# junghoseong/aircombat-selfplay

Measured on AMD Instinct MI355X. Metric: agent-steps/sec, higher is better.
Workload: dtype f32

## Files before the change

__graft_entry__.py:

```python
import os
import subprocess
import sys

ROOT = os.path.dirname(os.path.abspath(__file__))
PKG = os.path.join(ROOT, "aircombat-selfplay_amd")
HIPCC = os.environ.get("HIPCC", "/opt/rocm/bin/hipcc")


def _stale(out, srcs):
    if not os.path.exists(out):
        return True
    t = os.path.getmtime(out)
    return any(os.path.getmtime(s) > t for s in srcs if os.path.exists(s))


HIP_FLAGS = ["--offload-arch=gfx950", "-O3", "-std=c++17",
             "-fno-hip-fp32-correctly-rounded-divide-sqrt", "-fgpu-flush-denormals-to-zero",
             "-fno-slp-vectorize"]


def build_hip(force=False):
    csrc = os.path.join(PKG, "csrc")
    src = os.path.join(csrc, "aircombat.hip")
    gen = os.path.join(ROOT, "tools", "gen_split_tick.py")
    if subprocess.run([sys.executable, gen, "--check"]).returncode != 0:
        subprocess.check_call([sys.executable, gen], stdout=subprocess.DEVNULL)
    deps = [os.path.join(csrc, f) for f in sorted(os.listdir(csrc))] + [
        os.path.join(ROOT, "include", "aircombat.h"), os.path.join(ROOT, "include", "aircombat_buffer.h"), os.path.join(ROOT, "include", "aircombat_epoch.h"), os.path.join(ROOT, "include", "aircombat_rollout.h"),
        os.path.join(ROOT, "include", "aircombat_rollout_share.h"), os.path.join(ROOT, "include", "aircombat_eval.h"), os.path.join(ROOT, "include", "aircombat_league.h"), os.path.join(ROOT, "include", "aircombat_record.h"), os.path.join(ROOT, "include", "aircombat_spawn.h"), os.path.join(ROOT, "include", "aircombat_mutual.h"),
        os.path.join(ROOT, "tools", "check_exec_restore.py"), os.path.join(ROOT, "tools", "check_hidden_loads.py"),
        os.path.join(ROOT, "tools", "check_shuffle_discipline.py"), gen, os.path.abspath(__file__)]
    out = os.path.join(PKG, "libaircombat_hip.so")
    if force or _stale(out, deps):
        srcs = [os.path.join(csrc, f) for f in sorted(os.listdir(csrc)) if f.endswith((".hip", ".hpp"))]
        lint = subprocess.run([sys.executable, os.path.join(ROOT, "tools", "check_shuffle_discipline.py")] + srcs, capture_output=True, text=True)
        if lint.returncode != 0:
            raise RuntimeError("shuffle on the right of a short-circuit operator in the HIP sources:\n" + lint.stdout)
        bdir = os.path.join(PKG, "build")
        os.makedirs(bdir, exist_ok=True)
        asm = os.path.join(bdir, "aircombat_gfx950.s")
        subprocess.check_call([HIPCC] + HIP_FLAGS + ["--cuda-device-only", "-S", "-o", asm, src], stderr=subprocess.DEVNULL)
        lint = subprocess.run([sys.executable, os.path.join(ROOT, "tools", "check_exec_restore.py"), asm], capture_output=True, text=True)
        if lint.returncode != 0:
            raise RuntimeError("gfx950 code-generation hazard in the HIP extension, refusing to build it:\n" + lint.stdout)
        lint = subprocess.run([sys.executable, os.path.join(ROOT, "tools", "check_hidden_loads.py"), asm], capture_output=True, text=True)
        if lint.returncode != 0:
            raise RuntimeError("a hand-placed action-row load has its registers touched before its wait, refusing to build:\n" + lint.stdout)
        tmp = out + ".tmp"
        subprocess.check_call([HIPCC] + HIP_FLAGS + ["-fPIC", "-shared", "-o", tmp, src, "-lhsa-runtime64"])
        os.replace(tmp, out)
    return out


def build_oracle(force=False):
    out = os.path.join(ROOT, "oracle", "_build", "liboracle.so")
    srcs = [os.path.join(ROOT, "oracle", f) for f in
            ("f16_fdm.c", "geodesy.c", "combat_env.c", "state_bridge.c", "bench_port.c", "lowlevel_actor.c", "f16_fdm.h", "geodesy.h", "combat_env.h", "f16_tables.h")]
    if force or _stale(out, srcs):
        subprocess.check_call(["make", "-C", os.path.join(ROOT, "oracle")] + (["-B"] if force else []), stdout=subprocess.DEVNULL)
    return out


def build():
    build_hip()
    build_oracle()
    if ROOT not in sys.path:
        sys.path.insert(0, ROOT)
    import aircombat_selfplay_amd as pkg
    pkg.load_library()


def smoke():
    if ROOT not in sys.path:
        sys.path.insert(0, ROOT)
    import numpy as np
    import aircombat_selfplay_amd as pkg
    from oracle import oracle as O

    build_oracle()
    cfg = pkg.default_config("singlecombat")
    env = pkg.HipVecEnv(cfg, 8, device_id=0)
    ref = O.OracleVecEnv(O.config_from_ac(cfg), 8)
    obs = env.reset()
    robs = ref.reset()
    assert np.allclose(obs, robs, rtol=1e-4, atol=2e-4), np.abs(obs - robs).max()
    rng = np.random.default_rng(0)
    for _ in range(5):
        act = np.stack([rng.integers(0, n, size=(8, 2)) for n in (41, 41, 41, 30)], axis=-1).astype(np.float32)
        obs, rew, done, info = env.step(act)
        robs, rrew, rdone, _ = ref.step(act)
        assert np.allclose(obs, robs, rtol=1e-3, atol=1e-3), np.abs(obs - robs).max()
        assert np.allclose(rew, rrew, rtol=1e-3, atol=2e-3), np.abs(rew - rrew).max()
        assert (done == rdone).all()
    env.close()
    print("smoke ok: HIP step matches the oracle on 8 envs x 5 steps")


if __name__ == "__main__":
    build()
    if len(sys.argv) > 1 and sys.argv[1] == "smoke":
        smoke()
```

aircombat-selfplay_amd/capi.py:

```python
import ctypes as C
import os

AC_MAX_AGENTS = 8
AC_MAX_MISSILES_PER_AGENT = 4
AC_STATE_LEN = 128

AC_TASK_HEADING, AC_TASK_SINGLECOMBAT, AC_TASK_DODGE_MISSILE, AC_TASK_SHOOT_MISSILE, AC_TASK_MULTICOMBAT = 0, 1, 2, 3, 4
AC_TASK_SCENARIO1, AC_TASK_SCENARIO_NVN, AC_TASK_WVR, AC_TASK_MANEUVER = 5, 6, 7, 8
AC_ALIVE, AC_CRASH, AC_SHOTDOWN = 0, 1, 2
AC_CTL_FAST, AC_CTL_FP32 = 0, 1
AC_CENT_EXPLICIT, AC_CENT_ENV_SHARE = 0, 1
AC_POOL_PPO, AC_POOL_MAPPO = 0, 1


class HipExtensionMissing(RuntimeError):
    pass


(AC_BUF_OBS, AC_BUF_SHARE_OBS, AC_BUF_ACTIONS, AC_BUF_REWARDS, AC_BUF_MASKS, AC_BUF_BAD_MASKS, AC_BUF_ACTIVE_MASKS, AC_BUF_LOGP,
 AC_BUF_VALUES, AC_BUF_RETURNS, AC_BUF_RNN_ACTOR, AC_BUF_RNN_CRITIC, AC_BUF_ADVANTAGES, AC_BUF_NFIELDS) = range(14)
AC_EPOCH_FIELDS = ("obs", "share_obs", "actions", "masks", "active_masks", "action_log_probs", "advantages", "returns", "value_preds",
                   "rnn_states_actor", "rnn_states_critic")
AC_EPOCH_NFIELDS = len(AC_EPOCH_FIELDS)

# ... 156 lines not shown
               [(n, C.c_void_p) for n in ("rewards", "info", "stage", "spawned", "episode", "ret_acc", "wins", "played", "return_sum", "index")]


AC_MI_HIDDEN, AC_MI_WIDTH, AC_MI_MAX_ACT, AC_MI_MAX_OBS = 128, 256, 12, 128
AC_MI_WEIGHTS = ("p_w0", "p_b0", "p_w1", "p_b1", "p_w2", "p_b2", "q_w0", "q_b0", "q_w1", "q_b1", "q_w2", "q_b2")


class AcMiScore(C.Structure):
    _fields_ = [(n, C.c_int32) for n in ("E", "na", "T", "obs_dim", "act_dim", "hidden", "s0", "n", "add")] + [("ratio", C.c_float)] + \
               [(n, C.c_void_p) for n in ("OBS", "ACTIONS", "RNN_ACTOR", "REWARDS") + AC_MI_WEIGHTS + ("r_int", "mse")]


class AcMiGather(C.Structure):
    _fields_ = [(n, C.c_int32) for n in ("E", "na", "T", "obs_dim", "act_dim", "hidden", "m", "pad_")] + \
               [(n, C.c_void_p) for n in ("OBS", "ACTIONS", "RNN_ACTOR", "times", "X", "Y")]


AC_LATE_FRACTION_DEFAULT, AC_LATE_BUDGET_DEFAULT = 1.0, 400000


class AcLateStats(C.Structure):
    _fields_ = [("steps", C.c_int64), ("retries", C.c_int64), ("last_retries", C.c_int32), ("last_late", C.c_int32), ("retry_steps", C.c_int64), ("lowered", C.c_int64), ("disabled", C.c_int64), ("fraction", C.c_double), ("timed_steps", C.c_int64),
                ("copy_before_us", C.c_double), ("dispatch_us", C.c_double), ("copy_after_us", C.c_double), ("wait_us", C.c_double)]


AC_PPO_STAT_LOSS, AC_PPO_STAT_POLICY_LOSS, AC_PPO_STAT_VALUE_LOSS, AC_PPO_STAT_ENTROPY_LOSS, AC_PPO_STAT_RATIO_MEAN, AC_PPO_STAT_DENOMINATOR = range(6)
AC_PPO_NSTAT = 8

AC_PROBE_IN, AC_PROBE_OUT, AC_PROBE_MAX_ROWS = 6, 12, 1 << 22
AC_PROBE_OPS = ("fx_rcp", "fx_rsqrt", "fx_sqrt", "fx_sqrt_both", "fx_sincos", "atan2_fast", "acos_fast", "pow_pos", "tanh_fast", "atanh_fast",
                "sigmoid_f", "tanh_f", "atmosphere", "pitot", "vcas", "in_range_deg", "in_range_rad", "slew", "tef_kinematic", "seek",
                "posture_fn", "missile_height_f", "missile_height_d", "neu_height64", "locate", "locate_fast")
AC_PROBE_MSL_IN, AC_PROBE_MSL_TGT, AC_PROBE_MSL_OUT = 16, 7, 16
AC_PROBE_MSL_MAX_ROWS, AC_PROBE_MSL_MAX_TICKS, AC_PROBE_MSL_MAX_CELLS = 512, 4200, 1 << 19

_p = C.c_void_p
SIGNATURES = {
    "ac_state_field_name": (C.c_char_p, [C.c_int]),
    "ac_create": (C.c_int, [C.POINTER(AcConfig), C.c_int32, C.c_int32, C.c_uint64, C.POINTER(_p)]),
    "ac_destroy": (C.c_int, [_p]),
    "ac_obs_dim": (C.c_int, [_p]),
    "ac_act_dim": (C.c_int, [_p]),
    "ac_num_envs": (C.c_int, [_p]),
    "ac_num_agents": (C.c_int, [_p]),
    "ac_reset": (C.c_int, [_p, _p]),
    "ac_step": (C.c_int, [_p, _p, _p, _p, _p, _p]),
    "ac_host_buffers": (C.c_int, [_p, C.c_int32, C.POINTER(_p), C.POINTER(_p), C.POINTER(_p), C.POINTER(_p), C.POINTER(_p)]),
    "ac_host_set_detach": (C.c_int, [_p, C.c_int32]),
    "ac_host_set_free": (None, [_p, _p, _p, _p, _p]),
    "ac_step_host_async": (C.c_int, [_p, C.c_int32]),
    "ac_step_host_wait": (C.c_int, [_p]),
    "ac_step_host": (C.c_int, [_p, C.c_int32]),
    "ac_step_host_actions": (C.c_int, [_p, C.c_int32, _p, C.c_size_t]),
    "ac_late_config": (C.c_int, [_p, C.c_double, C.c_int32, C.c_int32, C.c_int32]),
    "ac_late_stats": (C.c_int, [_p, _p]),
    "ac_order_after": (C.c_int, [_p, _p]),
    "ac_order_before": (C.c_int, [_p, _p]),
    "ac_step_async_device": (C.c_int, [_p, _p]),
    "ac_device_buffers": (C.c_int, [_p, C.POINTER(_p), C.POINTER(_p), C.POINTER(_p), C.POINTER(_p), C.POINTER(_p)]),
    "ac_stream": (_p, [_p]),
    "ac_dispatch_path": (C.c_char_p, [_p]),
    "ac_sync": (C.c_int, [_p]),
    "ac_get_state": (C.c_int, [_p, C.c_int32, C.c_int32, C.POINTER(C.c_double)]),
    "ac_set_state": (C.c_int, [_p, C.c_int32, C.c_int32, C.POINTER(C.c_double)]),
    "ac_set_status": (C.c_int, [_p, C.c_int32, C.c_int32, C.c_int32]),
    "ac_get_entity": (C.c_int, [_p, C.c_int32, C.c_int32, C.POINTER(C.c_double)]),
    "ac_get_missile": (C.c_int, [_p, C.c_int32, C.c_int32, C.c_int32, C.POINTER(C.c_double)]),
    "ac_get_missile_target": (C.c_int, [_p, C.c_int32, C.c_int32, C.c_int32, C.POINTER(C.c_int32)]),
    "ac_timing_begin": (C.c_int, [_p]),
    "ac_timing_end": (C.c_int, [_p, C.POINTER(C.c_float)]),
    "ac_step_timed_device": (C.c_int, [_p, _p, C.POINTER(C.c_float), C.POINTER(C.c_float)]),
    "ac_state_checksum": (C.c_int, [_p, C.POINTER(C.c_uint64)]),
    "ac_munitions_in_flight": (C.c_int, [_p, C.POINTER(C.c_int32)]),
    "ac_seed_envs": (C.c_int, [_p, _p]),
    "ac_get_heading_state": (C.c_int, [_p, C.c_int32, _p]),
    "ac_pin_host_buffer": (C.c_int, [_p, _p, C.c_int64]),
    "ac_unpin_host_buffer": (C.c_int, [_p, _p]),
    "ac_load_controller": (C.c_int, [_p, _p, C.c_int64]),
    "ac_split_f16x2": (C.c_int, [_p, C.c_int64, _p, _p]),
    "ac_split_bf16x3": (C.c_int, [_p, C.c_int64, _p, _p, _p]),
    "ac_controller_precision": (C.c_int, [_p]),
    "ac_controller_forward": (C.c_int, [C.c_int32, C.c_int32, _p, C.c_int64, C.c_int64, _p, _p, _p, _p]),
    "ac_selftest_missile_walk": (C.c_int, [C.c_int32, _p]),
    "ac_probe_math": (C.c_int, [_p, C.c_int32, C.c_int64, _p, _p]),
    "ac_probe_missile": (C.c_int, [_p, C.c_int32, C.c_int32, C.c_int32, C.c_int32, _p, _p, _p]),
    "ac_get_controller_state": (C.c_int, [_p, C.c_int32, C.c_int32, _p, _p]),
    "ac_set_controller_state": (C.c_int, [_p, C.c_int32, C.c_int32, _p]),
    "ac_snapshot_bytes": (C.c_int, [_p, C.POINTER(C.c_int64)]),
    "ac_snapshot_header": (C.c_int, [_p, _p]),
    "ac_snapshot_save": (C.c_int, [_p, _p]),
    "ac_snapshot_load": (C.c_int, [_p, _p]),
    "ac_snapshot_save_host": (C.c_int, [_p, _p, C.c_int64]),
    "ac_snapshot_load_host": (C.c_int, [_p, _p, C.c_int64]),
    "ac_clone_envs": (C.c_int, [_p, _p, _p, C.c_int32]),
    "ac_snapshot_load_envs": (C.c_int, [_p, _p, _p, C.c_int32]),
    "ac_get_obs": (C.c_int, [_p, _p]),
    "ac_snapshot_checksum": (C.c_int, [_p, C.POINTER(C.c_uint64)]),
    "ac_policy_blob_floats": (C.c_int, [_p, C.POINTER(C.c_int64), C.POINTER(C.c_int64)]),
    "ac_policy_create": (C.c_int, [C.c_int32, _p, C.POINTER(_p)]),
    "ac_policy_destroy": (C.c_int, [_p]),
    "ac_policy_load": (C.c_int, [_p, _p, C.c_int64, _p, C.c_int64]),
    "ac_policy_load_device": (C.c_int, [_p, _p, _p, C.c_int64, _p, C.c_int64]),
    "ac_policy_load_refused": (C.c_int, [_p, _p, C.POINTER(C.c_int32), C.POINTER(C.c_int32)]),
    "ac_policy_packed": (C.c_int, [_p, C.c_int32, C.POINTER(_p), C.POINTER(C.c_int64)]),
    "ac_policy_get_actions": (C.c_int, [_p, _p, _p, _p, _p, _p, _p, C.c_int32, C.c_uint64, C.c_uint64, _p, _p, _p, _p, _p]),
    "ac_policy_draw_host": (C.c_int, [C.c_uint64, C.c_uint64, C.c_int64, C.c_int64, C.c_int32, _p]),
# ... 170 lines not shown
```

aircombat-selfplay_amd/csrc/aircombat.hip:

```cpp
#include <hip/hip_runtime.h>
#include <stdint.h>
#include <stdio.h>
#include <string.h>
#include <string>
#include <vector>
#include <cmath>
#include <algorithm>
#include <chrono>
#include "../../include/aircombat.h"
#include "../../include/aircombat_buffer.h"
#include "clk_stamps.hpp"
#include "f16_device.hpp"
#include "f16_split.hpp"

using f16::State;
using f16::Derived;
using f16::Tab;
using f16::clampf;

#define AC_F_FIELDS(X)                                                                                           \
  X(vx) X(vy) X(vz) X(q0) X(q1) X(q2) X(q3) X(wp) X(wq) X(wr) X(hv1x) X(hv1y) X(hv1z) X(hv2x) X(hv2y) X(hv2z)   \
  X(ha1x) X(ha1y) X(ha1z) X(wdx) X(wdy) X(wdz) X(aix) X(aiy) X(aiz) X(bax) X(bay) X(baz) X(da) X(de) X(dr)       \
  X(thr) X(pin_r) X(pin_p) X(pin_y) X(pi_r) X(pi_p) X(pi_y) X(tef) X(ail) X(elev) X(sbdeg) X(alpha) X(mach)      \
  X(qc) X(vg) X(ap) X(aq) X(ar) X(npx) X(npy) X(npz) X(n1) X(n2) X(n2norm) X(ff) X(tank0) X(tank1)
// ... 2063 lines not shown
    const size_t Npad = ((size_t)h->N + 63) / 64 * 64;
    const size_t act_bytes = (sizeof(float) * Npad * h->act_dim + 63) / 64 * 64;
    HIP_OK(hipHostMalloc((void**)&hs.act, act_bytes + sizeof(int) * late::HDR_WORDS, hipHostMallocDefault));
    hs.hdr = reinterpret_cast<int*>(reinterpret_cast<char*>(hs.act) + act_bytes);
    memset(hs.hdr, 0, sizeof(int) * late::HDR_WORDS);
    hs.tag = 0; hs.plain_rows = false;
    HIP_OK(hipHostMalloc((void**)&hs.obs, sizeof(float) * Npad * h->obs_dim, hipHostMallocDefault));
    HIP_OK(hipHostMalloc((void**)&hs.rew, sizeof(float) * Npad, hipHostMallocDefault));
    HIP_OK(hipHostMalloc((void**)&hs.done, Npad, hipHostMallocDefault));
    HIP_OK(hipHostMalloc((void**)&hs.info, sizeof(int) * (Npad / h->A), hipHostMallocDefault));
    memset(hs.act, 0, sizeof(float) * Npad * h->act_dim); memset(hs.obs, 0, sizeof(float) * Npad * h->obs_dim);
    memset(hs.rew, 0, sizeof(float) * Npad); memset(hs.done, 0, Npad); memset(hs.info, 0, sizeof(int) * (Npad / h->A));
    h->have_hs[set] = true;
  }
  if (actions) *actions = hs.act;
  if (obs) *obs = hs.obs;
  if (rewards) *rewards = hs.rew;
  if (dones) *dones = hs.done;
  if (info) *info = hs.info;
  return 0;
}
int ac_host_set_detach(ac_env_t* h, int32_t set) {
  if (!h || set < 0 || set >= AC_HOST_SETS || !h->have_hs[set]) return fail("ac_host_set_detach: no such set");
  if (host_entry(h)) return -1;
  HIP_OK(hipSetDevice(h->device));
  HIP_OK(hipStreamSynchronize(h->stream));
  h->have_hs[set] = false;
  memset(&h->hs[set], 0, sizeof h->hs[set]);
  return 0;
}
void ac_host_set_free(void* actions, void* obs, void* rewards, void* dones, void* info) {
  (void)hipHostFree(actions); (void)hipHostFree(obs); (void)hipHostFree(rewards); (void)hipHostFree(dones); (void)hipHostFree(info);
}
int ac_step_host_async(ac_env_t* h, int32_t set) {
  if (!h || set < 0 || set >= AC_HOST_SETS) return fail("ac_step_host_async: bad argument");
  if (!h->have_hs[set]) return fail("ac_step_host_async: call ac_host_buffers for this set first");
  HIP_OK(hipSetDevice(h->device));
  return host_step(h, set);
}
int ac_step_host_wait(ac_env_t* h) {
  if (!h) return fail("ac_step_host_wait: null handle");
  if (h->aql.in_flight) {
    if (aql_settle(h)) return -1;
  } else {
    HIP_OK(hipStreamSynchronize(h->stream));
    h->stream_dirty = false;
  }
  return check_nonfinite(h, "ac_step_host_wait");
}
int ac_step_host(ac_env_t* h, int32_t set) {
  if (ac_step_host_async(h, set)) return -1;
  return ac_step_host_wait(h);
}
int ac_step_host_actions(ac_env_t* h, int32_t set, const float* actions, size_t n_floats) {
  if (!h || !actions || set < 0 || set >= AC_HOST_SETS) return fail("ac_step_host_actions: bad argument");
  if (!h->have_hs[set]) return fail("ac_step_host_actions: call ac_host_buffers for this set first");
  if (n_floats != (size_t)h->N * h->act_dim) return fail("ac_step_host_actions: n_floats is not num_envs * num_agents * act_dim");
  HIP_OK(hipSetDevice(h->device));
  h->late_set = -1;
  if (host_step(h, set, actions)) return -1;
  const int ls = h->late_set;
  std::chrono::steady_clock::time_point t0;
  if (ls >= 0 && h->late_timing) t0 = std::chrono::steady_clock::now();
  const int rc = ac_step_host_wait(h);
  if (ls >= 0) {
    ac_late_stats_t& st = h->late_stats;
    if (h->late_timing) st.wait_us += std::chrono::duration<double, std::micro>(std::chrono::steady_clock::now() - t0).count();
    st.last_retries = *(volatile int*)&h->hs[ls].hdr[late::HDR_RETRIES];
    st.retries += st.last_retries;
    st.retry_steps += st.last_retries != 0;
    st.steps += 1;
    h->late_win_steps += 1;
    h->late_win_retry += st.last_retries != 0;
    if (h->late_win_steps == AC_LATE_WINDOW) {
      if (h->late_win_retry > AC_LATE_WINDOW_MAX_RETRY_STEPS) {
        h->late_fraction -= 0.25;
        st.lowered += 1;
        if (h->late_fraction <= 0.0) { h->late_fraction = 0.0; h->late_off = true; st.disabled = 1; }
      }
      h->late_win_steps = h->late_win_retry = 0;
    }
    st.fraction = h->late_fraction;
    h->late_set = -1;
  }
  return rc;
}
int ac_late_config(ac_env_t* h, double fraction, int32_t budget, int32_t delay_us, int32_t timing) {
  if (!h) return fail("ac_late_config: null handle");
  if (fraction > 1.0 || budget > (1 << 24)) return fail("ac_late_config: fraction above 1 or budget above 2^24 tries");
  if (host_entry(h)) return -1;
  if (fraction >= 0.0) { h->late_fraction = fraction; h->late_off = false; h->late_stats.disabled = 0; h->late_win_steps = h->late_win_retry = 0; }
  if (budget >= 0) h->late_budget = budget;
  if (delay_us >= 0) h->late_delay_us = delay_us;
  if (timing >= 0) h->late_timing = timing != 0;
  return 0;
}
int ac_late_stats(ac_env_t* h, ac_late_stats_t* out) {
  if (!h || !out) return fail("ac_late_stats: null argument");
  *out = h->late_stats;
  out->fraction = h->late_fraction;
  return 0;
}

int ac_order_after(ac_env_t* h, void* producer_stream) {
  if (!h) return fail("ac_order_after: null handle");
  if (host_entry(h)) return -1;
  HIP_OK(hipSetDevice(h->device));
  HIP_OK(hipEventRecord(h->ev_order, (hipStream_t)producer_stream));
  HIP_OK(hipStreamWaitEvent(h->stream, h->ev_order, 0));
  return 0;
}
int ac_order_before(ac_env_t* h, void* consumer_stream) {
  if (!h) return fail("ac_order_before: null handle");
  if (host_entry(h)) return -1;
  HIP_OK(hipSetDevice(h->device));
  HIP_OK(hipEventRecord(h->ev_order, h->stream));
  HIP_OK(hipStreamWaitEvent((hipStream_t)consumer_stream, h->ev_order, 0));
  return 0;
}

int ac_step_async_device(ac_env_t* h, const float* d_actions) {
  if (!h) return fail("ac_step_async_device: null handle");
  if (host_entry(h)) return -1;
  HIP_OK(hipSetDevice(h->device));
  return launch_step(h, d_actions);
}
int ac_device_buffers(ac_env_t* h, float** d_actions, float** d_obs, float** d_rewards, uint8_t** d_dones, int32_t** d_info) {
  if (!h) return fail("ac_device_buffers: null handle");
  if (d_actions) *d_actions = h->d_actions;
  if (d_obs) *d_obs = h->dp.obs;
  if (d_rewards) *d_rewards = h->dp.rew;
  if (d_dones) *d_dones = h->dp.done;
  if (d_info) *d_info = h->dp.info;
  return 0;
}
void* ac_stream(ac_env_t* h) {
  if (!h) return nullptr;
  (void)host_entry(h);
// ... 496 lines not shown
```

aircombat-selfplay_amd/vec_env.py:

```python
import ctypes as C
import os
import sys

import numpy as np

from .capi import (AcConfig, AC_STATE_LEN, AC_TASK_HEADING, AC_TASK_SINGLECOMBAT, AC_TASK_SHOOT_MISSILE, AC_TASK_MULTICOMBAT, AC_TASK_SCENARIO1,
                   AC_TASK_SCENARIO_NVN, AC_CTL_FAST, AC_CTL_FP32, load_library)
from . import capi
from .config import config_from_yaml, default_config
from .snapshot import EnvSnapshot, MultiSnapshot, SnapshotMismatch, check_compatible, decode_header

DONE_MESSAGES = {
    0: "", 1: "altitude is too low", 2: "is on an extreme state", 3: "acceleration is too high", 4: "has been shot down",
    5: "has crashed", 6: "mission completed", 7: "step limits", 8: "unreached heading",
}


class _Box:

    def __init__(self, low, high, shape):
        self.low = np.full(shape, low, dtype=np.float32)
        self.high = np.full(shape, high, dtype=np.float32)
        self.shape = tuple(shape)
        self.dtype = np.float32

    def __repr__(self):
        return f"Box({self.low.min()}, {self.high.max()}, {self.shape}, float32)"


class _MultiDiscrete:
    def __init__(self, nvec):
        self.nvec = np.asarray(nvec, dtype=np.int64)
        self.shape = self.nvec.shape
        self.dtype = np.int64

    def __repr__(self):
        return f"MultiDiscrete({self.nvec.tolist()})"


class _Discrete:
    def __init__(self, n):
        self.n = int(n)
        self.shape = ()
        self.dtype = np.int64


class _Tuple(tuple):
    pass


class LazyInfos:

    __slots__ = ("_codes",)

    def __init__(self, codes, snapshot=False):
        self._codes = np.array(codes, copy=True) if snapshot else codes

    def __len__(self):
        return len(self._codes)

    shape = property(lambda self: (len(self._codes),))
    ndim, dtype = 1, np.dtype(object)

# ... 96 lines not shown

class HipVecEnv:

    def __init__(self, config, num_envs, device_id=0, seed=0, lib=None, copy=True, controller_precision=None):
        if not isinstance(config, AcConfig):
            raise TypeError("config must be an AcConfig (see config_from_yaml / default_config)")
        if controller_precision is not None:
            prec = _controller_precision_id(controller_precision)
            config = AcConfig.from_buffer_copy(config)
            config.controller_precision = prec
        self.lib = lib or load_library()
        self.config = config
        self.copy = bool(copy)
        self.num_envs = int(num_envs)
        self.num_agents = int(config.n_agents)
        handle = C.c_void_p()
        self.lib.check(self.lib.ac_create(C.byref(config), self.num_envs, int(device_id), int(seed), C.byref(handle)), "ac_create")
        self._h = handle
        self._device_id = int(device_id)
        self.closed = False
        self.waiting = False
        self.obs_dim = self.lib.ac_obs_dim(self._h)
        self.act_dim = self.lib.ac_act_dim(self._h)
        Box, MultiDiscrete, Discrete, Tuple = _spaces()
        self.observation_space = Box(low=-10, high=10.0, shape=(self.obs_dim,))
        self.hierarchical = bool(config.hierarchical)
        if config.task == AC_TASK_HEADING:
            self._seed_heading(int(seed))
        if self.hierarchical:
            w = np.fromfile(CONTROLLER_WEIGHTS, dtype=np.float32)
            self.lib.check(self.lib.ac_load_controller(self._h, w.ctypes.data, int(w.size)), "ac_load_controller")
        if self.hierarchical and config.task in (AC_TASK_SCENARIO1, AC_TASK_SCENARIO_NVN):
            self.action_space = Tuple([MultiDiscrete([3, 5, 3]), MultiDiscrete([2, 2, 2, 2])])
        elif self.hierarchical and (config.legacy_obs or config.task == AC_TASK_SHOOT_MISSILE):
            self.action_space = Tuple([MultiDiscrete([3, 5, 3]), Discrete(2)])
        elif self.hierarchical:
            self.action_space = MultiDiscrete([3, 5, 3])
        elif config.task == AC_TASK_SHOOT_MISSILE or config.legacy_obs and config.task == AC_TASK_MULTICOMBAT:
            self.action_space = Tuple([MultiDiscrete([41, 41, 41, 30]), Discrete(2)])
        elif config.task in (AC_TASK_SCENARIO1, AC_TASK_SCENARIO_NVN):
            self.action_space = Tuple([MultiDiscrete([41, 41, 41, 30]), MultiDiscrete([2, 2, 2, 2])])
        else:
            self.action_space = MultiDiscrete([41, 41, 41, 30])
        self._sets = []
        for k in range(2):
            self._add_set()
        self._cur = 0
        self._pending = None
        self._staging = None
        self._actions = self._sets[0]["actions"]
        self._results = [self._result(st) for st in self._sets]
        self._step_host = self.lib.ac_step_host_actions
        self._ref0 = self._refs(self._sets[0])

    def _add_set(self):
        k = len(self._sets)
        E, A = self.num_envs, self.num_agents
        ptrs = [C.c_void_p() for _ in range(5)]
        self.lib.check(self.lib.ac_host_buffers(self._h, k, *[C.byref(p) for p in ptrs]), "ac_host_buffers")
        owner = _HostSetOwner(self.lib, ptrs)

        def arr(ptr, shape, typestr):
            return np.asarray(_Mapped(owner, ptr.value, shape, typestr))

        st = {"actions": arr(ptrs[0], (E, A, self.act_dim), "<f4"), "owner": owner, "index": k,
              "out": (arr(ptrs[1], (E, A, self.obs_dim), "<f4"), arr(ptrs[2], (E, A, 1), "<f4"), arr(ptrs[3], (E, A, 1), "|b1"),
                      arr(ptrs[4], (E,), "<i4"))}
        self._extend_set(st)
        self._sets.append(st)
        return st

    def _extend_set(self, st):
        """Hook for subclasses that hand out one more array per set (HipShareVecEnv: the share_obs view)."""

    def _held(self, st):
        return self._refs(st) != self._ref0

    @staticmethod
    def _refs(st):
        t = st["out"]
        if len(t) == 4:
            return sys.getrefcount(t[0]), sys.getrefcount(t[1]), sys.getrefcount(t[2]), sys.getrefcount(t[3])
        return sys.getrefcount(t[0]), sys.getrefcount(t[1]), sys.getrefcount(t[2]), sys.getrefcount(t[3]), sys.getrefcount(t[4])

    def _next_set(self):
        if not self.copy:
            self._cur ^= 1
            return self._sets[self._cur], False
        n = len(self._sets)
        for i in range(1, n + 1):
            st = self._sets[(self._cur + i) % n]
            if not self._held(st):
                self._cur = st["index"]
                return st, False
        if n < RING_SETS:
            st = self._add_set()
            self._results.append(self._result(st))
            self._cur = st["index"]
            return st, False
        if self._staging is None:
            self._staging = self._add_set()
            self._sets.pop()
        return self._staging, True

    def seed(self, seed=None):
        if seed is not None and self.config.task == AC_TASK_HEADING:
            self._seed_heading(int(seed))

    def _seed_heading(self, seed):
        st = np.zeros((self.num_envs, 4), dtype=np.uint64)
        m = (1 << 64) - 1
        for i in range(self.num_envs):
            b = np.random.PCG64(seed + 1000 * i).state["state"]
            st[i] = (b["state"] >> 64, b["state"] & m, b["inc"] >> 64, b["inc"] & m)
        self.lib.check(self.lib.ac_seed_envs(self._h, st.ctypes.data), "ac_seed_envs")

    def reset(self):
        self._assert_not_closed()
        obs = np.empty((self.num_envs, self.num_agents, self.obs_dim), dtype=np.float32)
        self.lib.check(self.lib.ac_reset(self._h, obs.ctypes.data), "ac_reset")
        return obs

    def _hand_over(self, actions):
        st, staged = self._next_set()
        dst = st["actions"]
        a = actions if isinstance(actions, np.ndarray) else np.asarray(actions, dtype=np.float32)
        if a.shape != dst.shape:
            a = a.reshape(dst.shape)
        np.copyto(dst, a)
        return st, staged

    def step_async(self, actions):
        self._assert_not_closed()
        self._pending = self._hand_over(actions)
        self.lib.check(self.lib.ac_step_host_async(self._h, self._pending[0]["index"]), "ac_step_host_async")
        self.waiting = True

    def step_wait(self):
        self._assert_not_closed()
        self.lib.check(self.lib.ac_step_host_wait(self._h), "ac_step_host_wait")
        self.waiting = False
        st, staged = self._pending
        return self._returned(st, staged)

    def _returned(self, st, staged):
        if not self.copy:
            return self._results[st["index"]]
        return self._fresh(st) if staged else self._owned(st)

    def _result(self, st):
        o = st["out"]
        return o[0], o[1], o[2], LazyInfos(o[3])

    def _owned(self, st):
        o = st["out"]
        return o[0], o[1], o[2], LazyInfos(o[3])

    def _fresh(self, st):
        o = st["out"]
        return o[0].copy(), o[1].copy(), o[2].copy(), LazyInfos(o[3], snapshot=True)

    def step(self, actions):
        assert not self.closed, "Trying to operate on a HipVecEnv after calling close()"
        st, staged = self._next_set()
        a = actions
        if not (isinstance(a, np.ndarray) and a.dtype == np.float32 and a.flags.c_contiguous):
            a = np.ascontiguousarray(actions, dtype=np.float32)
        if a.size != self._actions.size:
            a = a.reshape(self._actions.shape)
        try:
            addr = C.addressof(C.c_char.from_buffer(a))
        except (TypeError, ValueError):
            addr = a.ctypes.data
        if self._step_host(self._h, st["index"], addr, a.size) != 0:
            self.lib.check(-1, "ac_step_host_actions")
        return self._returned(st, staged)

    def render(self, mode="txt", filepath="./JSBSimRecording.txt.acmi", env=0):
        from . import acmi
        if mode != "txt":
            raise NotImplementedError
        self._assert_not_closed()
        cfg = self.config
        step = int(self.get_state(env, 0)[self._ix("cur_step")])
        if not getattr(self, "_acmi_started", False):
            with open(filepath, mode="w", encoding="utf-8-sig") as f:
                f.write(acmi.HEADER)
            self._acmi_started, self._acmi = True, acmi.FrameWriter(cfg, self.num_agents)
        w = self._acmi
        entities = [self.get_entity(env, a) for a in range(self.num_agents)]
        slots = []
        for a in range(self.num_agents):
            ms = [self.get_missile(env, a, k) for k in range(w.n_slots[a])]
            slots.append([(m[0], m[11], m[1], m[2], m[3], m[7], m[8]) for m in ms])
        chaff = None
        if w.has_chaff:
            chaff = []
            for a in range(self.num_agents):
                st = self.get_state(env, a)
                chaff.append((int(st[self._ix("x_n_ch")]),
                              tuple((int(st[self._ix(f"x_ch_status{q}")]), int(st[self._ix(f"x_ch_mult{q}")])) for q in range(2))))
        with open(filepath, mode="a", encoding="utf-8-sig") as f:
            f.write(w.frame(step, entities, slots, chaff))

    def record(self, envs=None, frames=1024):
        from .recorder import FlightRecorder
        self._assert_not_closed()
        rec = FlightRecorder(self, envs=envs, frames=frames)
        try:
            rec.attach()
        except Exception:
            rec.close()
            raise
        return rec

    def stop_recording(self):
        self._assert_not_closed()
        self.lib.check(self.lib.ac_recorder_detach(self._h), "ac_recorder_detach")
        self._recorder = None

    @property
    def recorder(self):
        return getattr(self, "_recorder", None)

    def spawn_curriculum(self, angles=None, init_states=None, mode="fixed", sample="at", win_return=None, window=20, win_rate=0.9, seed=0):
        from .spawn import SpawnCurriculum
        self._assert_not_closed()
        return SpawnCurriculum(self, angles=angles, init_states=init_states, mode=mode, sample=sample, win_return=win_return, window=window,
                               win_rate=win_rate, seed=seed)

    def stop_curriculum(self):
        self._assert_not_closed()
        cur = getattr(self, "_curriculum", None)
        if cur is not None:
            cur.close()
        self.lib.check(self.lib.ac_spawn_detach(self._h), "ac_spawn_detach")

    @property
    def curriculum(self):
        return getattr(self, "_curriculum", None)

    def _ix(self, name):
        if not hasattr(self, "_names"):
            self._names = self.lib.state_field_names()
        return self._names.index(name)

    def close(self):
        if self.closed:
            return
        for ref in list(getattr(self, "_recorders", [])):
            rec = ref()
            if rec is not None:
                rec.close()
        self._recorder = None
        cur = getattr(self, "_curriculum", None)
        if cur is not None:
            cur.close()
        if self.copy:
            for st in self._sets:
                if self._held(st):
                    self.lib.check(self.lib.ac_host_set_detach(self._h, st["index"]), "ac_host_set_detach")
                    st["owner"].detached = True
        self._sets, self._results, self._staging, self._pending = [], [], None, None
        self._actions = None
        self.lib.ac_destroy(self._h)
        self._h = None
        self.closed = True

    def _assert_not_closed(self):
        assert not self.closed, "Trying to operate on a HipVecEnv after calling close()"

    def __del__(self):
        try:
            self.close()
        except Exception:
            pass

    def device_tensors(self):
        import torch

        ptrs = [C.c_void_p() for _ in range(5)]
        self.lib.check(self.lib.ac_device_buffers(self._h, *[C.byref(p) for p in ptrs]), "ac_device_buffers")
        E, A = self.num_envs, self.num_agents

        def view(ptr, shape, typestr):
            holder = type("_DeviceBuffer", (), {})()
            holder.__cuda_array_interface__ = {"shape": shape, "typestr": typestr, "data": (ptr.value, False), "version": 2}
            return torch.as_tensor(holder, device="cuda")

        act = view(ptrs[0], (E, A, self.act_dim), "<f4")
        obs = view(ptrs[1], (E, A, self.obs_dim), "<f4")
        rew = view(ptrs[2], (E, A, 1), "<f4")
        done = view(ptrs[3], (E, A, 1), "|u1")
        info = view(ptrs[4], (E, 4), "<i4")
        return act, obs, rew, done, info

    def step_device(self, d_actions_ptr=None, stream=None):
        if stream is not None:
            raw = getattr(stream, "cuda_stream", stream)
            self.lib.check(self.lib.ac_order_after(self._h, raw), "ac_order_after")
        self.lib.check(self.lib.ac_step_async_device(self._h, d_actions_ptr), "ac_step_async_device")
        if stream is not None:
            self.lib.check(self.lib.ac_order_before(self._h, raw), "ac_order_before")

    def sync(self):
        self.lib.check(self.lib.ac_sync(self._h), "ac_sync")

    def get_state(self, env, agent):
        out = (C.c_double * AC_STATE_LEN)()
        self.lib.check(self.lib.ac_get_state(self._h, env, agent, out), "ac_get_state")
# ... 303 lines not shown
```

include/aircombat.h:

```cpp
#ifndef AIRCOMBAT_H
#define AIRCOMBAT_H
#include <stddef.h>
#include <stdint.h>
#ifdef __cplusplus
extern "C" {
#endif

#define AC_MAX_AGENTS 8
#define AC_MAX_MISSILES_PER_AGENT 4

enum {
  AC_TASK_HEADING = 0,
  AC_TASK_SINGLECOMBAT = 1,
  AC_TASK_DODGE_MISSILE = 2,
  AC_TASK_SHOOT_MISSILE = 3,
  AC_TASK_SCENARIO1 = 5,
  AC_TASK_SCENARIO_NVN = 6,
  AC_TASK_WVR = 7,
  AC_TASK_MANEUVER = 8,
  AC_TASK_MULTICOMBAT = 4
};
enum { AC_ALIVE = 0, AC_CRASH = 1, AC_SHOTDOWN = 2 };
enum { AC_DONE_NONE = 0, AC_DONE_LOW_ALTITUDE = 1, AC_DONE_EXTREME_STATE = 2, AC_DONE_OVERLOAD = 3, AC_DONE_SHOTDOWN = 4,
       AC_DONE_CRASHED = 5, AC_DONE_MISSION_COMPLETE = 6, AC_DONE_TIMEOUT = 7, AC_DONE_UNREACH_HEADING = 8 };
// ... 10 lines not shown
  int32_t agent_interaction_steps;
  int32_t max_steps;
  double center_lon, center_lat, center_alt;
  double altitude_limit;
  double acc_limit_x, acc_limit_y, acc_limit_z;
  ac_init_state_t init[AC_MAX_AGENTS];
  int32_t num_missiles[AC_MAX_AGENTS];
  double posture_scale;  int32_t posture_potential;
  double altitude_scale; int32_t altitude_potential;
  double event_scale;    int32_t event_potential;
  double missile_posture_scale;
  double shoot_penalty_scale; int32_t shoot_penalty_potential;
  double alt_safe, alt_danger, alt_kv;
  double max_attack_angle, max_attack_distance; int32_t min_attack_interval;
  int32_t use_artillery;
  double heading_scale; int32_t heading_potential;
  double max_heading_increment, max_altitude_increment, max_velocities_u_increment, check_interval;
  int32_t legacy_obs;
  int32_t rwr;
  int32_t use_baseline;
  int32_t hierarchical;
  int32_t approach;
  int32_t controller_precision;
} ac_config_t;
enum { AC_CTL_FAST = 0, AC_CTL_FP32 = 1 };

typedef struct ac_env ac_env_t;

#define AC_STATE_LEN 128
const char* ac_state_field_name(int i);

int ac_create(const ac_config_t* cfg, int32_t n_envs, int32_t device_id, uint64_t seed, ac_env_t** out);
int ac_destroy(ac_env_t* h);
int ac_obs_dim(const ac_env_t* h);
int ac_act_dim(const ac_env_t* h);
int ac_num_envs(const ac_env_t* h);
int ac_num_agents(const ac_env_t* h);

int ac_reset(ac_env_t* h, float* obs);
int ac_step(ac_env_t* h, const float* actions, float* obs, float* rewards, uint8_t* dones, int32_t* info);

#define AC_INFO_STEP(w) ((int32_t)((uint32_t)(w) & 0xFFFFu))
#define AC_INFO_DONE_CODE(w) ((int32_t)(((uint32_t)(w) >> 16) & 0xFFu))
#define AC_INFO_TURN_COUNTS(w) ((int32_t)(((uint32_t)(w) >> 24) & 0x7Fu))
#define AC_INFO_WAS_RESET(w) ((int32_t)((uint32_t)(w) >> 31))
#define AC_HOST_SETS 8
int ac_host_buffers(ac_env_t* h, int32_t set, float** actions, float** obs, float** rewards, uint8_t** dones, int32_t** info);
int ac_host_set_detach(ac_env_t* h, int32_t set);
void ac_host_set_free(void* actions, void* obs, void* rewards, void* dones, void* info);
int ac_step_host_async(ac_env_t* h, int32_t set);
int ac_step_host_wait(ac_env_t* h);
int ac_step_host(ac_env_t* h, int32_t set);
int ac_step_host_actions(ac_env_t* h, int32_t set, const float* actions, size_t n_floats);
#define AC_LATE_FRACTION_DEFAULT 1.0
#define AC_LATE_BUDGET_DEFAULT 400000
#define AC_LATE_WINDOW 1024
#define AC_LATE_WINDOW_MAX_RETRY_STEPS 16
typedef struct {
  int64_t steps;
  int64_t retries;
  int32_t last_retries;
  int32_t last_late;
  int64_t retry_steps;
  int64_t lowered;
  int64_t disabled;
  double fraction;
  int64_t timed_steps;
  double copy_before_us, dispatch_us, copy_after_us, wait_us;
} ac_late_stats_t;
int ac_late_config(ac_env_t* h, double fraction, int32_t budget, int32_t delay_us, int32_t timing);
int ac_late_stats(ac_env_t* h, ac_late_stats_t* out);

int ac_step_async_device(ac_env_t* h, const float* d_actions);
int ac_device_buffers(ac_env_t* h, float** d_actions, float** d_obs, float** d_rewards, uint8_t** d_dones, int32_t** d_info);
void* ac_stream(ac_env_t* h);
const char* ac_dispatch_path(ac_env_t* h);
int ac_sync(ac_env_t* h);
int ac_order_after(ac_env_t* h, void* producer_stream);
int ac_order_before(ac_env_t* h, void* consumer_stream);

int ac_get_state(ac_env_t* h, int32_t env, int32_t agent, double* out );
int ac_set_state(ac_env_t* h, int32_t env, int32_t agent, const double* in );
int ac_set_status(ac_env_t* h, int32_t env, int32_t agent, int32_t status);
int ac_get_entity(ac_env_t* h, int32_t env, int32_t agent, double out[12]);
int ac_get_missile(ac_env_t* h, int32_t env, int32_t agent, int32_t k, double out[12]);
int ac_get_missile_target(ac_env_t* h, int32_t env, int32_t agent, int32_t k, int32_t* target);

int ac_state_checksum(ac_env_t* h, uint64_t* out);

int ac_munitions_in_flight(ac_env_t* h, int32_t* count);

int ac_seed_envs(ac_env_t* h, const uint64_t* states);
int ac_get_heading_state(ac_env_t* h, int32_t env, double out[8]);

int ac_pin_host_buffer(ac_env_t* h, void* ptr, int64_t bytes);
int ac_unpin_host_buffer(ac_env_t* h, void* ptr);

int ac_load_controller(ac_env_t* h, const float* weights, int64_t n);
int ac_get_controller_state(ac_env_t* h, int32_t env, int32_t agent, float* hidden, float* low_action);
int ac_set_controller_state(ac_env_t* h, int32_t env, int32_t agent, const float* hidden);
int ac_controller_precision(ac_env_t* h);
int ac_controller_forward(int32_t device_id, int32_t precision, const float* weights, int64_t n_weights,
                          int64_t n, const float* x, float* h, float* logits, int32_t* action);
int ac_split_f16x2(const float* x, int64_t n, float* hi, float* lo);
int ac_split_bf16x3(const float* x, int64_t n, float* b0, float* b1, float* b2);
int ac_selftest_missile_walk(int32_t device_id, int32_t* mismatches);
// ... 229 lines not shown
```

Measured before the change: 246.1 million.

## Add native C++ Python extension for VecEnv.step with split begin/wait host calls

Adds a CPython extension Stepper that does the whole step in C instead of the interpreter: it picks the host buffer set, checks the action buffer format, dispatches the step, builds the result tuple and waits with the GIL released. The HIP host step is split into begin and wait entry points so the result tuple is built while the GPU runs. The aim is to cut Python interpreter and ctypes overhead per step. The cost is a second compiled module, reference-count based detection of held sets that could misbehave, and a Python fallback when the extension is missing.

```diff
diff --git a/__graft_entry__.py b/__graft_entry__.py
--- a/__graft_entry__.py
+++ b/__graft_entry__.py
@@ -25,7 +25,7 @@
     gen = os.path.join(ROOT, "tools", "gen_split_tick.py")
     if subprocess.run([sys.executable, gen, "--check"]).returncode != 0:
         subprocess.check_call([sys.executable, gen], stdout=subprocess.DEVNULL)
-    deps = [os.path.join(csrc, f) for f in sorted(os.listdir(csrc))] + [
+    deps = [os.path.join(csrc, f) for f in sorted(os.listdir(csrc)) if not f.startswith("native_step")] + [
         os.path.join(ROOT, "include", "aircombat.h"), os.path.join(ROOT, "include", "aircombat_buffer.h"), os.path.join(ROOT, "include", "aircombat_epoch.h"), os.path.join(ROOT, "include", "aircombat_rollout.h"),
         os.path.join(ROOT, "include", "aircombat_rollout_share.h"), os.path.join(ROOT, "include", "aircombat_eval.h"), os.path.join(ROOT, "include", "aircombat_league.h"), os.path.join(ROOT, "include", "aircombat_record.h"), os.path.join(ROOT, "include", "aircombat_spawn.h"), os.path.join(ROOT, "include", "aircombat_mutual.h"),
         os.path.join(ROOT, "tools", "check_exec_restore.py"), os.path.join(ROOT, "tools", "check_hidden_loads.py"),
@@ -52,6 +52,24 @@
     return out
 
 
+def build_native(force=False):
+    import shutil
+    import sysconfig
+    csrc = os.path.join(PKG, "csrc")
+    srcs = [os.path.join(csrc, "native_step.cpp"), os.path.join(csrc, "native_step_pick.hpp")]
+    out = os.path.join(PKG, "_native_step" + sysconfig.get_config_var("EXT_SUFFIX"))
+    inc = sysconfig.get_paths()["include"]
+    cxx = os.environ.get("CXX") or shutil.which("g++") or shutil.which("c++") or shutil.which("clang++")
+    if not os.path.exists(os.path.join(inc, "Python.h")) or not cxx:
+        print(f"build: {'no Python.h in ' + inc if cxx else 'no host C++ compiler'}: the native VecEnv.step is not built, step() runs its Python path", file=sys.stderr)
+        return None
+    if force or _stale(out, srcs):
+        tmp = out + ".tmp"
+        subprocess.check_call([cxx, "-std=c++17", "-O2", "-fPIC", "-shared", "-fvisibility=hidden", "-I", inc, "-I", csrc, "-o", tmp, srcs[0]])
+        os.replace(tmp, out)
+    return out
+
+
 def build_oracle(force=False):
     out = os.path.join(ROOT, "oracle", "_build", "liboracle.so")
     srcs = [os.path.join(ROOT, "oracle", f) for f in
@@ -63,6 +81,7 @@
 
 def build():
     build_hip()
+    build_native()
     build_oracle()
     if ROOT not in sys.path:
         sys.path.insert(0, ROOT)
diff --git a/aircombat-selfplay_amd/capi.py b/aircombat-selfplay_amd/capi.py
--- a/aircombat-selfplay_amd/capi.py
+++ b/aircombat-selfplay_amd/capi.py
@@ -232,6 +232,8 @@
     "ac_step_host_wait": (C.c_int, [_p]),
     "ac_step_host": (C.c_int, [_p, C.c_int32]),
     "ac_step_host_actions": (C.c_int, [_p, C.c_int32, _p, C.c_size_t]),
+    "ac_step_host_actions_begin": (C.c_int, [_p, C.c_int32, _p, C.c_size_t]),
+    "ac_step_host_actions_wait": (C.c_int, [_p]),
     "ac_late_config": (C.c_int, [_p, C.c_double, C.c_int32, C.c_int32, C.c_int32]),
     "ac_late_stats": (C.c_int, [_p, _p]),
     "ac_order_after": (C.c_int, [_p, _p]),
diff --git a/aircombat-selfplay_amd/csrc/aircombat.hip b/aircombat-selfplay_amd/csrc/aircombat.hip
--- a/aircombat-selfplay_amd/csrc/aircombat.hip
+++ b/aircombat-selfplay_amd/csrc/aircombat.hip
@@ -2139,13 +2139,16 @@
   if (ac_step_host_async(h, set)) return -1;
   return ac_step_host_wait(h);
 }
-int ac_step_host_actions(ac_env_t* h, int32_t set, const float* actions, size_t n_floats) {
+int ac_step_host_actions_begin(ac_env_t* h, int32_t set, const float* actions, size_t n_floats) {
   if (!h || !actions || set < 0 || set >= AC_HOST_SETS) return fail("ac_step_host_actions: bad argument");
   if (!h->have_hs[set]) return fail("ac_step_host_actions: call ac_host_buffers for this set first");
   if (n_floats != (size_t)h->N * h->act_dim) return fail("ac_step_host_actions: n_floats is not num_envs * num_agents * act_dim");
   HIP_OK(hipSetDevice(h->device));
   h->late_set = -1;
-  if (host_step(h, set, actions)) return -1;
+  return host_step(h, set, actions);
+}
+int ac_step_host_actions_wait(ac_env_t* h) {
+  if (!h) return fail("ac_step_host_actions_wait: null handle");
   const int ls = h->late_set;
   std::chrono::steady_clock::time_point t0;
   if (ls >= 0 && h->late_timing) t0 = std::chrono::steady_clock::now();
@@ -2171,6 +2174,10 @@
     h->late_set = -1;
   }
   return rc;
+}
+int ac_step_host_actions(ac_env_t* h, int32_t set, const float* actions, size_t n_floats) {
+  if (ac_step_host_actions_begin(h, set, actions, n_floats)) return -1;
+  return ac_step_host_actions_wait(h);
 }
 int ac_late_config(ac_env_t* h, double fraction, int32_t budget, int32_t delay_us, int32_t timing) {
   if (!h) return fail("ac_late_config: null handle");
diff --git a/aircombat-selfplay_amd/csrc/native_step.cpp b/aircombat-selfplay_amd/csrc/native_step.cpp
--- /dev/null
+++ b/aircombat-selfplay_amd/csrc/native_step.cpp
@@ -0,0 +1,263 @@
+#define PY_SSIZE_T_CLEAN
+#include <Python.h>
+#include <structmember.h>
+
+#include <cstddef>
+#include <cstdint>
+
+#include "native_step_pick.hpp"
+
+namespace {
+
+using begin_fn = int (*)(void*, int32_t, const float*, size_t);
+using wait_fn = int (*)(void*);
+
+struct SetRec {
+  PyObject* out;
+  PyObject* result;
+  Py_ssize_t baseline[native_step::MAX_ARRAYS];
+};
+
+struct Stepper {
+  PyObject_HEAD
+  begin_fn begin;
+  wait_fn wait;
+  void* handle;
+  size_t n_floats;
+  int copy, share, n_arrays, n_sets;
+  SetRec sets[native_step::MAX_SETS];
+  PyObject* lazy_infos;
+  PyObject* check;
+};
+
+PyObject* g_cur_name = nullptr;
+PyObject* g_failed_name = nullptr;
+PyObject* g_minus_one = nullptr;
+
+void* address_arg(PyObject* o) { return PyLong_AsVoidPtr(o); }
+
+int stepper_init(PyObject* self_, PyObject* args, PyObject* kwds) {
+  Stepper* s = (Stepper*)self_;
+  static const char* names[] = {"begin", "wait", "handle", "n_floats", "copy", "share", "lazy_infos", "check", nullptr};
+  PyObject *b, *w, *h, *lazy, *check;
+  Py_ssize_t n;
+  int copy, share;
+  if (!PyArg_ParseTupleAndKeywords(args, kwds, "OOOnppOO", (char**)names, &b, &w, &h, &n, &copy, &share, &lazy, &check)) return -1;
+  void* bp = address_arg(b);
+  void* wp = address_arg(w);
+  void* hp = address_arg(h);
+  if (PyErr_Occurred()) return -1;
+  if (!bp || !wp || !hp || n <= 0 || !PyCallable_Check(lazy) || !PyCallable_Check(check)) {
+    PyErr_SetString(PyExc_ValueError, "Stepper: null address, empty batch or a non-callable");
+    return -1;
+  }
+  s->begin = (begin_fn)bp;
+  s->wait = (wait_fn)wp;
+  s->handle = hp;
+  s->n_floats = (size_t)n;
+  s->copy = copy;
+  s->share = share;
+  s->n_arrays = share ? 5 : 4;
+  Py_INCREF(lazy);
+  Py_XSETREF(s->lazy_infos, lazy);
+  Py_INCREF(check);
+  Py_XSETREF(s->check, check);
+  return 0;
+}
+
+void stepper_clear_sets(Stepper* s) {
+  const int n = s->n_sets;
+  s->n_sets = 0;
+  for (int k = 0; k < n; ++k) {
+    Py_CLEAR(s->sets[k].out);
+    Py_CLEAR(s->sets[k].result);
+  }
+}
+
+void stepper_dealloc(PyObject* self_) {
+  Stepper* s = (Stepper*)self_;
+  stepper_clear_sets(s);
+  Py_CLEAR(s->lazy_infos);
+  Py_CLEAR(s->check);
+  Py_TYPE(self_)->tp_free(self_);
+}
+
+PyObject* stepper_add_set(PyObject* self_, PyObject* const* args, Py_ssize_t nargs) {
+  Stepper* s = (Stepper*)self_;
+  if (nargs != 2 || !PyTuple_CheckExact(args[0]) || PyTuple_GET_SIZE(args[0]) != s->n_arrays) {
+    PyErr_SetString(PyExc_TypeError, "add_set(out, result): out is the set's tuple of arrays");
+    return nullptr;
+  }
+  if (s->n_sets >= native_step::MAX_SETS) {
+    PyErr_SetString(PyExc_ValueError, "add_set: the ring is full");
+    return nullptr;
+  }
+  if (!s->copy && !PyTuple_CheckExact(args[1])) {
+    PyErr_SetString(PyExc_TypeError, "add_set: with copy=False result is the tuple step() returns for the set");
+    return nullptr;
+  }
+  SetRec& r = s->sets[s->n_sets];
+  Py_INCREF(args[0]);
+  r.out = args[0];
+  r.result = nullptr;
+  if (!s->copy) {
+    Py_INCREF(args[1]);
+    r.result = args[1];
+  }
+  for (int i = 0; i < s->n_arrays; ++i) r.baseline[i] = Py_REFCNT(PyTuple_GET_ITEM(r.out, i));
+  s->n_sets += 1;
+  Py_RETURN_NONE;
+}
+
+bool set_held(const Stepper* s, int k) {
+  const SetRec& r = s->sets[k];
+  Py_ssize_t now[native_step::MAX_ARRAYS];
+  for (int i = 0; i < s->n_arrays; ++i) now[i] = Py_REFCNT(PyTuple_GET_ITEM(r.out, i));
+  return native_step::held(now, r.baseline, s->n_arrays);
+}
+
+PyObject* stepper_held(PyObject* self_, PyObject* arg) {
+  Stepper* s = (Stepper*)self_;
+  const long k = PyLong_AsLong(arg);
+  if (k == -1 && PyErr_Occurred()) return nullptr;
+  if (k < 0 || k >= s->n_sets) {
+    PyErr_SetString(PyExc_IndexError, "held: no such set");
+    return nullptr;
+  }
+  return PyBool_FromLong(set_held(s, (int)k));
+}
+
+PyObject* stepper_clear(PyObject* self_, PyObject*) {
+  stepper_clear_sets((Stepper*)self_);
+  Py_RETURN_NONE;
+}
+
+PyObject* build_result(Stepper* s, int k) {
+  SetRec& r = s->sets[k];
+  if (!s->copy) {
+    Py_INCREF(r.result);
+    return r.result;
+  }
+  PyObject* infos = PyObject_CallFunctionObjArgs(s->lazy_infos, PyTuple_GET_ITEM(r.out, 3), nullptr);
+  if (!infos) return nullptr;
+  PyObject* t = PyTuple_New(s->share ? 5 : 4);
+  if (!t) {
+    Py_DECREF(infos);
+    return nullptr;
+  }
+  static const int plain[3] = {0, 1, 2}, shared[4] = {0, 4, 1, 2};
+  const int* order = s->share ? shared : plain;
+  const int n = s->share ? 4 : 3;
+  for (int i = 0; i < n; ++i) {
+    PyObject* a = PyTuple_GET_ITEM(r.out, order[i]);
+    Py_INCREF(a);
+    PyTuple_SET_ITEM(t, i, a);
+  }
+  PyTuple_SET_ITEM(t, n, infos);
+  return t;
+}
+
+PyObject* raise_library_error(Stepper* s) {
+  PyObject* r = PyObject_CallFunctionObjArgs(s->check, g_minus_one, g_failed_name, nullptr);
+  if (r) {
+    Py_DECREF(r);
+    PyErr_SetString(PyExc_RuntimeError, "ac_step_host_actions failed");
+  }
+  return nullptr;
+}
+
+PyObject* stepper_step(PyObject* self_, PyObject* const* args, Py_ssize_t nargs) {
+  Stepper* s = (Stepper*)self_;
+  if (nargs != 2) {
+    PyErr_SetString(PyExc_TypeError, "step(env, actions)");
+    return nullptr;
+  }
+  PyObject* env = args[0];
+  PyObject* actions = args[1];
+  PyObject* cur_obj = PyObject_GetAttr(env, g_cur_name);
+  if (!cur_obj) return nullptr;
+  const long cur_l = PyLong_AsLong(cur_obj);
+  Py_DECREF(cur_obj);
+  if (cur_l == -1 && PyErr_Occurred()) return nullptr;
+  const int cur = (cur_l < 0 || cur_l >= native_step::MAX_SETS) ? -1 : (int)cur_l;
+  int k;
+  if (!s->copy) k = s->n_sets >= 2 ? native_step::pick_alternate(cur) : native_step::FALLBACK;
+  else k = native_step::pick_ring(cur, s->n_sets, [s](int i) { return set_held(s, i); });
+  if (k == native_step::FALLBACK) Py_RETURN_NONE;
+  if (!PyObject_CheckBuffer(actions)) Py_RETURN_NONE;
+  Py_buffer view;
+  if (PyObject_GetBuffer(actions, &view, PyBUF_C_CONTIGUOUS | PyBUF_FORMAT) != 0) {
+    PyErr_Clear();
+    Py_RETURN_NONE;
+  }
+  if (!native_step::fast_actions(view.format, view.itemsize, view.len, s->n_floats)) {
+    PyBuffer_Release(&view);
+    Py_RETURN_NONE;
+  }
+  const int rc_begin = s->begin(s->handle, (int32_t)k, (const float*)view.buf, s->n_floats);
+  PyBuffer_Release(&view);
+  PyObject* idx = PyLong_FromLong(k);
+  const int set_rc = idx ? PyObject_SetAttr(env, g_cur_name, idx) : -1;
+  Py_XDECREF(idx);
+  if (rc_begin != 0) {
+    PyErr_Clear();
+    return raise_library_error(s);
+  }
+  PyObject* result = set_rc == 0 ? build_result(s, k) : nullptr;
+  PyObject *et = nullptr, *ev = nullptr, *tb = nullptr;
+  if (!result) PyErr_Fetch(&et, &ev, &tb);
+  int rc;
+  Py_BEGIN_ALLOW_THREADS
+  rc = s->wait(s->handle);
+  Py_END_ALLOW_THREADS
+  if (!result) {
+    PyErr_Restore(et, ev, tb);
+    return nullptr;
+  }
+  if (rc != 0) {
+    Py_DECREF(result);
+    return raise_library_error(s);
+  }
+  return result;
+}
+
+PyMethodDef stepper_methods[] = {
+    {"step", (PyCFunction)(void (*)(void))stepper_step, METH_FASTCALL, "step(env, actions) -> result tuple, or None: take the Python path"},
+    {"add_set", (PyCFunction)(void (*)(void))stepper_add_set, METH_FASTCALL, "add_set(out, result): the next set of the ring; records the baseline counts"},
+    {"held", stepper_held, METH_O, "held(k): does anybody outside hold an array of set k"},
+    {"clear", stepper_clear, METH_NOARGS, "drop every set (close())"},
+    {nullptr, nullptr, 0, nullptr}};
+
+PyMemberDef stepper_members[] = {{"n_sets", T_INT, offsetof(Stepper, n_sets), READONLY, "sets in the ring"}, {nullptr, 0, 0, 0, nullptr}};
+
+PyTypeObject StepperType = {PyVarObject_HEAD_INIT(nullptr, 0)};
+
+PyModuleDef moduledef = {PyModuleDef_HEAD_INIT, "_native_step", "VecEnv.step without the interpreter (csrc/native_step.cpp)", -1, nullptr, nullptr, nullptr, nullptr, nullptr};
+
+}
+
+PyMODINIT_FUNC PyInit__native_step(void) {
+  StepperType.tp_name = "_native_step.Stepper";
+  StepperType.tp_basicsize = sizeof(Stepper);
+  StepperType.tp_flags = Py_TPFLAGS_DEFAULT;
+  StepperType.tp_doc = "Stepper(begin, wait, handle, n_floats, copy, share, lazy_infos, check)";
+  StepperType.tp_new = PyType_GenericNew;
+  StepperType.tp_init = stepper_init;
+  StepperType.tp_dealloc = stepper_dealloc;
+  StepperType.tp_methods = stepper_methods;
+  StepperType.tp_members = stepper_members;
+  if (PyType_Ready(&StepperType) < 0) return nullptr;
+  g_cur_name = PyUnicode_InternFromString("_cur");
+  g_failed_name = PyUnicode_InternFromString("ac_step_host_actions");
+  g_minus_one = PyLong_FromLong(-1);
+  if (!g_cur_name || !g_failed_name || !g_minus_one) return nullptr;
+  PyObject* m = PyModule_Create(&moduledef);
+  if (!m) return nullptr;
+  Py_INCREF(&StepperType);
+  if (PyModule_AddObject(m, "Stepper", (PyObject*)&StepperType) < 0) {
+    Py_DECREF(&StepperType);
+    Py_DECREF(m);
+    return nullptr;
+  }
+  return m;
+}
diff --git a/aircombat-selfplay_amd/csrc/native_step_pick.hpp b/aircombat-selfplay_amd/csrc/native_step_pick.hpp
--- /dev/null
+++ b/aircombat-selfplay_amd/csrc/native_step_pick.hpp
@@ -0,0 +1,36 @@
+#pragma once
+#include <cstddef>
+
+namespace native_step {
+
+constexpr int MAX_SETS = 8;
+constexpr int MAX_ARRAYS = 5;
+constexpr int FALLBACK = -1;
+
+inline int pick_alternate(int cur) { return (cur == 0 || cur == 1) ? (cur ^ 1) : FALLBACK; }
+
+template <class Count>
+inline bool held(const Count* now, const Count* baseline, int n_arrays) {
+  for (int i = 0; i < n_arrays; ++i)
+    if (now[i] != baseline[i]) return true;
+  return false;
+}
+
+template <class IsHeld>
+inline int pick_ring(int cur, int n_sets, IsHeld is_held) {
+  if (n_sets < 1 || n_sets > MAX_SETS || cur < 0 || cur >= n_sets) return FALLBACK;
+  for (int i = 1; i <= n_sets; ++i) {
+    const int k = (cur + i) % n_sets;
+    if (!is_held(k)) return k;
+  }
+  return FALLBACK;
+}
+
+inline bool fast_actions(const char* format, std::ptrdiff_t itemsize, std::ptrdiff_t len_bytes, std::size_t n_floats) {
+  if (!format || itemsize != (std::ptrdiff_t)sizeof(float)) return false;
+  if (format[0] == '@' || format[0] == '=' || format[0] == '<') ++format;
+  if (format[0] != 'f' || format[1] != '\0') return false;
+  return len_bytes >= 0 && (std::size_t)len_bytes == n_floats * sizeof(float);
+}
+
+}
diff --git a/aircombat-selfplay_amd/vec_env.py b/aircombat-selfplay_amd/vec_env.py
--- a/aircombat-selfplay_amd/vec_env.py
+++ b/aircombat-selfplay_amd/vec_env.py
@@ -9,6 +9,11 @@
 from . import capi
 from .config import config_from_yaml, default_config
 from .snapshot import EnvSnapshot, MultiSnapshot, SnapshotMismatch, check_compatible, decode_header
+
+try:
+    from . import _native_step
+except ImportError:
+    _native_step = None
 
 DONE_MESSAGES = {
     0: "", 1: "altitude is too low", 2: "is on an extreme state", 3: "acceleration is too high", 4: "has been shot down",
@@ -211,6 +216,18 @@
         self._results = [self._result(st) for st in self._sets]
         self._step_host = self.lib.ac_step_host_actions
         self._ref0 = self._refs(self._sets[0])
+        self._native = None
+        if _native_step is not None and os.environ.get("AIRCOMBAT_NATIVE_STEP", "1") != "0":
+            dll = self.lib.dll
+            self._native = _native_step.Stepper(C.cast(dll.ac_step_host_actions_begin, C.c_void_p).value,
+                                                C.cast(dll.ac_step_host_actions_wait, C.c_void_p).value, self._h.value,
+                                                self._actions.size, self.copy, len(self._sets[0]["out"]) == 5, LazyInfos, self.lib.check)
+            for st in self._sets:
+                self._native_add(st)
+
+    def _native_add(self, st):
+        if self._native is not None:
+            self._native.add_set(st["out"], self._results[st["index"]])
 
     def _add_set(self):
         k = len(self._sets)
@@ -255,6 +272,7 @@
         if n < RING_SETS:
             st = self._add_set()
             self._results.append(self._result(st))
+            self._native_add(st)
             self._cur = st["index"]
             return st, False
         if self._staging is None:
@@ -320,13 +338,22 @@
         return o[0].copy(), o[1].copy(), o[2].copy(), LazyInfos(o[3], snapshot=True)
 
     def step(self, actions):
+        native = self._native
+        if native is not None:
+            res = native.step(self, actions)
+            if res is not None:
+                return res
         assert not self.closed, "Trying to operate on a HipVecEnv after calling close()"
-        st, staged = self._next_set()
         a = actions
         if not (isinstance(a, np.ndarray) and a.dtype == np.float32 and a.flags.c_contiguous):
             a = np.ascontiguousarray(actions, dtype=np.float32)
         if a.size != self._actions.size:
             a = a.reshape(self._actions.shape)
+        if native is not None and a is not actions:
+            res = native.step(self, a)
+            if res is not None:
+                return res
+        st, staged = self._next_set()
         try:
             addr = C.addressof(C.c_char.from_buffer(a))
         except (TypeError, ValueError):
@@ -415,6 +442,9 @@
         cur = getattr(self, "_curriculum", None)
         if cur is not None:
             cur.close()
+        if getattr(self, "_native", None) is not None:
+            self._native.clear()
+        self._native = None
         if self.copy:
             for st in self._sets:
                 if self._held(st):
diff --git a/include/aircombat.h b/include/aircombat.h
--- a/include/aircombat.h
+++ b/include/aircombat.h
@@ -86,6 +86,8 @@
 int ac_step_host_wait(ac_env_t* h);
 int ac_step_host(ac_env_t* h, int32_t set);
 int ac_step_host_actions(ac_env_t* h, int32_t set, const float* actions, size_t n_floats);
+int ac_step_host_actions_begin(ac_env_t* h, int32_t set, const float* actions, size_t n_floats);
+int ac_step_host_actions_wait(ac_env_t* h);
 #define AC_LATE_FRACTION_DEFAULT 1.0
 #define AC_LATE_BUDGET_DEFAULT 400000
 #define AC_LATE_WINDOW 1024
```

After: 258.5 million, median of 6. 5.0% higher.
